# ydchen0806/CLC

Hardware: AMD Instinct MI355X
Metric: images/sec fwd+bwd @256x256 bs8; bpp+PSNR parity vs ref (higher is better)
Workload: dtype f32

## Files before the change

clc_amd/csrc/conv_igemm.hip:

```cpp
#include "common.h"
#ifndef CLC_PF32
#define CLC_PF32 3
#endif

namespace {
#include "conv_common.h"
template <int BM, int BN, int WM, int WN, bool TR>
__global__ __launch_bounds__(64 * WM * WN, (64 * WM * WN) >= 512 ? 4 : ((64 * WM * WN) >= 256 ? 2 : 4))
void conv_igemm_kernel(const ConvParams p) {
  constexpr int NT = 64 * WM * WN;
  constexpr int TM = BM / WM / 32, TN = BN / WN / 32;
  constexpr int A_P = BM * 8 / NT, B_P = BN * 8 / NT;
  static_assert(TM >= 1 && TN >= 1 && A_P * NT == BM * 8 && B_P * NT == BN * 8, "tile");
  extern __shared__ __attribute__((aligned(16))) float smem[];
  float* As = smem;
  float* Bs = smem + 2 * BM * LD;

  const int tid = threadIdx.x, lane = tid & 63, wave = tid >> 6;
  const int wm = wave / WN, wn = wave % WN;
  const int m0 = blockIdx.x * BM, n0 = blockIdx.y * BN;
  const int cls = blockIdx.z, ph = cls >> 1, pw = cls & 1;
  const bool half = p.transposed && p.stride == 2;
  const int DH = half ? p.OH / 2 : p.OH, DW = half ? p.OW / 2 : p.OW;
  const TapGrid tg = make_taps(p, ph, pw);
// ... 431 lines not shown
    dma_a(buf ^ 1); dma_b(buf ^ 1);
    __builtin_amdgcn_s_setprio(0);
    read_frag(buf, 1, af[1], bf[1]);
    mfma_group(af[0], bf[0]);
    read_frag(buf, 2, af[0], bf[0]);
    mfma_group(af[1], bf[1]);
    read_frag(buf, 3, af[1], bf[1]);
    mfma_group(af[0], bf[0]);
    mfma_group(af[1], bf[1]);
    asm volatile("s_waitcnt vmcnt(0)" ::: "memory");
    __syncthreads();
    read_frag(buf ^ 1, 0, af[0], bf[0]);
  }

  if (ksp > 1) {
    float* dst = p.partial + ((size_t)(cls * ksp + sk) * p.M) * p.Cout;
#pragma unroll
    for (int i = 0; i < TM; ++i)
#pragma unroll
      for (int j = 0; j < TN; ++j) {
        const int co = n0 + wn * (BN / WN) + j * 32 + lr;
        const int row0 = m0 + wm * (BM / WM) + i * 32 + 4 * hh;
        if (co >= p.Cout) continue;
#pragma unroll
        for (int r = 0; r < 16; ++r) dst[(size_t)(row0 + (r & 3) + 8 * (r >> 2)) * p.Cout + co] = acc[i][j][r];
      }
    return;
  }
  if (p.reg_epi) {
    const RegEpi re = make_reg_epi(p);
#pragma unroll
    for (int i = 0; i < TM; ++i)
#pragma unroll
      for (int j = 0; j < TN; ++j) {
        const int co = n0 + wn * (BN / WN) + j * 32 + lr;
        epilogue_regs(p, re, acc[i][j], bsel ? bsel[co] : 0.f, (unsigned)(m0 + wm * (BM / WM) + i * 32 + 4 * hh), co);
      }
    return;
  }
  constexpr int LDC = BN + 4;
  float* Cs = smem;
  __syncthreads();
  {
    const int col = lane & 31, rhalf = 4 * (lane >> 5);
#pragma unroll
    for (int i = 0; i < TM; ++i)
#pragma unroll
      for (int j = 0; j < TN; ++j)
#pragma unroll
        for (int r = 0; r < 16; ++r)
          Cs[(wm * (BM / WM) + i * 32 + (r & 3) + 8 * (r >> 2) + rhalf) * LDC + wn * (BN / WN) + j * 32 + col] = acc[i][j][r];
  }
  __syncthreads();
  if (p.vec_epi) {
    for (int e = tid; e < BM * BN / 4; e += NT) {
      const int row = e / (BN / 4), cc = (e - row * (BN / 4)) * 4;
      const int m = m0 + row, co = n0 + cc;
      if (m < p.M && co < p.Cout) epilogue_store4(p, bsel, *reinterpret_cast<const f32x4*>(Cs + row * LDC + cc), m, co, DH, DW, ph, pw);
    }
    return;
  }
  for (int e = tid; e < BM * BN; e += NT) {
    const int row = e / BN, cc = e - row * BN;
    const int m = m0 + row, co = n0 + cc;
    if (m < p.M && co < p.Cout) epilogue_store(p, Cs[row * LDC + cc], bsel ? bsel[co] : 0.f, m, co, DH, DW, ph, pw);
  }
}

template <int KS>
__global__ __launch_bounds__(256, 2)
void conv_igemm_n16_kernel(const ConvParams p) {
  constexpr int BM = 256, NT = 256, A_P = 8;
  extern __shared__ __attribute__((aligned(16))) float smem[];
  float* As = smem;
  float* Bs = smem + 2 * BM * BK;
  const int tid = threadIdx.x, lane = tid & 63, wave = tid >> 6;
  const int m0 = blockIdx.x * BM;
  const int DH = p.OH, DW = p.OW;
  const __amdgpu_buffer_rsrc_t xr = __builtin_amdgcn_make_buffer_rsrc(const_cast<float*>(p.x), 0, p.x_bytes, 0x00020000);
  const __amdgpu_buffer_rsrc_t wr = __builtin_amdgcn_make_buffer_rsrc(const_cast<float*>(p.w), 0, p.w_bytes, 0x00020000);
  unsigned a_base[A_P], a_mask[A_P];
  int a_c4[A_P];
#pragma unroll
  for (int i = 0; i < A_P; ++i) {
    const int r = (tid + i * NT) >> 3;
    const RowState rs = make_row<false>(p, m0 + r, DH, DW, 0, 0);
    a_c4[i] = ((tid & 7) ^ ((r >> 1) & 7)) * 4;
    unsigned mask = 0;
#pragma unroll
    for (int j = 0; j < KS; ++j)
#pragma unroll
      for (int q = 0; q < KS; ++q) {
        const int iy = rs.y0 + j, ix = rs.x0 + q;
        mask |= (rs.ok && (unsigned)iy < (unsigned)p.H && (unsigned)ix < (unsigned)p.W) ? (1u << (j * 3 + q)) : 0u;
      }
    a_mask[i] = mask;
    a_base[i] = ((unsigned)(rs.base + rs.y0 * p.W + rs.x0) * (unsigned)p.ldx + (unsigned)a_c4[i]) * 4u;
  }
  const int b_r = tid >> 3, b_c4 = ((tid & 7) ^ ((b_r >> 1) & 7)) * 4;
  const bool b_ok = tid < 128 && b_r < p.Cout;
  const unsigned b_base = ((unsigned)b_r * (unsigned)p.ldw + (unsigned)b_c4) * 4u;
  const int wave_row = wave * 8;

  f32x4 acc[4];
#pragma unroll
  for (int rb = 0; rb < 4; ++rb) acc[rb] = (f32x4){0.f, 0.f, 0.f, 0.f};
  const int total = KS * KS * p.kc_tiles;
  int tj = 0, ti = 0, kc = 0;
  auto advance = [&]() {
    const int kc1 = kc + 1;
    const bool w1 = kc1 == p.kc_tiles;
    kc = w1 ? 0 : kc1;
    const int ti1 = ti + (w1 ? 1 : 0);
    const bool w2 = ti1 == KS;
    ti = w2 ? 0 : ti1;
    tj += w2 ? 1 : 0;
  };
  unsigned s_bit, s_adelta, s_bdelta; int s_cleft; bool s_en;
  auto set_fetch = [&](bool en) {
    s_en = en;
    s_bit = 1u << (tj * 3 + ti);
    s_cleft = p.Cin - kc * BK;
    s_adelta = (unsigned)((tj * p.W + ti) * p.ldx + kc * BK) * 4u;
    s_bdelta = (unsigned)((tj * KS + ti) * p.Cin + kc * BK) * 4u;
  };
  auto dma_tile = [&](int buf) {
#pragma unroll
    for (int i = 0; i < A_P; ++i) {
      const bool ok = s_en && (a_mask[i] & s_bit) != 0u && a_c4[i] < s_cleft;
      dma16(xr, As + (buf * BM + wave_row + i * (NT / 8)) * BK, ok ? a_base[i] + s_adelta : kOOB);
    }
    if (wave < 2) dma16(wr, Bs + (buf * 16 + wave_row) * BK, (s_en && b_ok && b_c4 < s_cleft) ? b_base + s_bdelta : kOOB);
  };
  set_fetch(true);
  dma_tile(0);
  asm volatile("s_waitcnt vmcnt(0)" ::: "memory");
  __syncthreads();
  const int li = lane & 15, g = lane >> 4, sw = (li >> 1) & 7;
  int fo[2];
#pragma unroll
  for (int t = 0; t < 2; ++t) fo[t] = ((4 * t + g) ^ sw) * 4;
  for (int it = 0; it < total; ++it) {
    const int buf = it & 1;
    advance();
    set_fetch(it + 1 < total);
    dma_tile(buf ^ 1);
    const float* Ab = As + (buf * BM + wave * 64 + li) * BK;
    const float* Bb = Bs + (buf * 16 + li) * BK;
#pragma unroll
    for (int t = 0; t < 2; ++t) {
      f32x4 a[4];
#pragma unroll
      for (int rb = 0; rb < 4; ++rb) a[rb] = *reinterpret_cast<const f32x4*>(Ab + rb * 16 * BK + fo[t]);
      const f32x4 b = *reinterpret_cast<const f32x4*>(Bb + fo[t]);
#pragma unroll
      for (int s = 0; s < 4; ++s)
#pragma unroll
        for (int rb = 0; rb < 4; ++rb) acc[rb] = __builtin_amdgcn_mfma_f32_16x16x4f32(a[rb][s], b[s], acc[rb], 0, 0, 0);
    }
    asm volatile("s_waitcnt vmcnt(0)" ::: "memory");
    __syncthreads();
  }
  const int co = li;
  if (co < p.Cout) {
    const float bv = p.bias ? p.bias[co] : 0.f;
#pragma unroll
    for (int rb = 0; rb < 4; ++rb)
#pragma unroll
      for (int r = 0; r < 4; ++r) {
        const int m = m0 + wave * 64 + rb * 16 + 4 * g + r;
        if (m < p.M) epilogue_store(p, acc[rb][r], bv, m, co, DH, DW, 0, 0);
      }
  }
}

__device__ __forceinline__ void wait_vm(int n) {
  if (n >= 63) asm volatile("s_waitcnt vmcnt(63) lgkmcnt(0)" ::: "memory");
  else if (n == 35) asm volatile("s_waitcnt vmcnt(35) lgkmcnt(0)" ::: "memory");
  else if (n == 19) asm volatile("s_waitcnt vmcnt(19) lgkmcnt(0)" ::: "memory");
  else asm volatile("s_waitcnt vmcnt(3) lgkmcnt(0)" ::: "memory");
}
template <int OP>
__global__ __launch_bounds__(512, 4)
void conv_igemm_p1x1_kernel(const ConvParams p, int tiles_m, int tiles_n) {
  constexpr int BM = 128, BN = 64, NT = 512, NS = 3, SLOT = (BM + BN) * BK;
  constexpr int P = 3;
  extern __shared__ __attribute__((aligned(16))) float smem[];
  const int tid = threadIdx.x, lane = tid & 63, wave = tid >> 6;
  const int wm = wave >> 1, wn = wave & 1;
  const int G = gridDim.x;
  const __amdgpu_buffer_rsrc_t xr = __builtin_amdgcn_make_buffer_rsrc(const_cast<float*>(p.x), 0, p.x_bytes, 0x00020000);
  const __amdgpu_buffer_rsrc_t wr = __builtin_amdgcn_make_buffer_rsrc(const_cast<float*>(p.w), 0, p.w_bytes, 0x00020000);

  unsigned a_lane[2], b_lane;
  int a_c4[2], b_c4;
#pragma unroll
  for (int i = 0; i < 2; ++i) {
    const int r = (tid + i * NT) >> 3;
    a_c4[i] = ((tid & 7) ^ ((r >> 1) & 7)) * 4;
    a_lane[i] = ((unsigned)r * (unsigned)p.ldx + (unsigned)a_c4[i]) * 4u;
  }
  {
    const int r = tid >> 3;
    b_c4 = ((tid & 7) ^ ((r >> 1) & 7)) * 4;
    b_lane = ((unsigned)r * (unsigned)p.ldw + (unsigned)b_c4) * 4u;
  }
  const int wave_row = wave * 8;
  float* bias_s = smem + NS * SLOT;
  for (int i = tid; i < p.Cout; i += NT) bias_s[i] = p.bias ? p.bias[i] : 0.f;
  const int my_mt = (tiles_m - (int)blockIdx.x + G - 1) / G;
  const int total = my_mt * tiles_n * p.kc_tiles;

  struct Cur { int mt, nt, kt, n; };
  auto step = [&](Cur& c) {
    const int kt1 = c.kt + 1;
    const bool w1 = kt1 == p.kc_tiles;
    c.kt = w1 ? 0 : kt1;
    const int nt1 = c.nt + (w1 ? 1 : 0);
    const bool w2 = nt1 == tiles_n;
    c.nt = w2 ? 0 : nt1;
    c.mt += w2 ? G : 0;
    ++c.n;
  };
  auto dma = [&](int slot, const Cur& c) {
    const bool en = c.n < total;
    const int cleft = p.Cin - c.kt * BK;
    const unsigned ao = ((unsigned)(c.mt * BM) * (unsigned)p.ldx + (unsigned)(c.kt * BK)) * 4u;
    const unsigned bo = ((unsigned)(c.nt * BN) * (unsigned)p.ldw + (unsigned)(c.kt * BK)) * 4u;
    float* base = smem + slot * SLOT;
#pragma unroll
    for (int i = 0; i < 2; ++i) dma16(xr, base + (wave_row + i * 64) * BK, (en && a_c4[i] < cleft) ? a_lane[i] + ao : kOOB);
    dma16(wr, base + (BM + wave_row) * BK, (en && b_c4 < cleft) ? b_lane + bo : kOOB);
  };

  const int lr = lane & 31, hh = lane >> 5, sw = (lr >> 1) & 7;
  int fo[4];
#pragma unroll
  for (int t8 = 0; t8 < 4; ++t8) fo[t8] = ((2 * t8 + hh) ^ sw) * 4;
  f32x4 af[2], bf[2];
  auto read_frag = [&](int slot, int t8, f32x4& a, f32x4& b) {
    const float* base = smem + slot * SLOT;
    a = *reinterpret_cast<const f32x4*>(base + (wm * 32 + lr) * BK + fo[t8]);
    if (OP == 1) a = a * a;
    b = *reinterpret_cast<const f32x4*>(base + (BM + wn * 32 + lr) * BK + fo[t8]);
  };
  f32x16 acc;
#pragma unroll
  for (int r = 0; r < 16; ++r) acc[r] = 0.f;
  auto mfma4 = [&](const f32x4& a, const f32x4& b) {
#pragma unroll
    for (int ss = 0; ss < 4; ++ss) acc = __builtin_amdgcn_mfma_f32_32x32x2f32(a[ss], b[ss], acc, 0, 0, 0);
  };

  const RegEpi re = make_reg_epi(p);
  const int S = p.y_pre ? 32 : 16;
  auto epilogue = [&](int mt, int nt) {
    const int co = nt * BN + wn * 32 + lr;
    epilogue_regs(p, re, acc, bias_s[co], (unsigned)(mt * BM + wm * 32 + 4 * hh), co);
  };


  Cur cf{(int)blockIdx.x, 0, 0, 0}, cc = cf;
  dma(0, cf); step(cf);
  dma(1, cf); step(cf);
  asm volatile("s_waitcnt vmcnt(3) lgkmcnt(0)" ::: "memory");
  __builtin_amdgcn_s_barrier();
  int slot = 0, slot2 = 2, e_prev = 0;
  for (int s = 0; s < total; ++s) {
    dma(slot2, cf); step(cf);
    read_frag(slot, 0, af[0], bf[0]);
    read_frag(slot, 1, af[1], bf[1]);
    mfma4(af[0], bf[0]);
    read_frag(slot, 2, af[0], bf[0]);
    mfma4(af[1], bf[1]);
    read_frag(slot, 3, af[1], bf[1]);
    mfma4(af[0], bf[0]);
    mfma4(af[1], bf[1]);
    const bool last = cc.kt == p.kc_tiles - 1;
    if (last) {
      epilogue(cc.mt, cc.nt);
#pragma unroll
      for (int r = 0; r < 16; ++r) acc[r] = 0.f;
    }
    const int e_cur = last ? 1 : 0;
    wait_vm(P + S * (e_prev + e_cur));
    __builtin_amdgcn_s_barrier();
    e_prev = e_cur;
    step(cc);
    slot = slot == 2 ? 0 : slot + 1;
    slot2 = slot2 == 2 ? 0 : slot2 + 1;
  }
  asm volatile("s_waitcnt vmcnt(0)" ::: "memory");
}

template <int BN, bool TR, int KW, int PF, bool OPS>
__global__ __launch_bounds__(64 * KW, KW == 8 ? (PF >= 2 ? 1 : 4) : 4)
void conv_igemm_splitk_kernel(const ConvParams p) {
  constexpr int BM = 32, TN = BN / 32;
  extern __shared__ __attribute__((aligned(16))) float smem[];
  const int tid = threadIdx.x, lane = tid & 63, wave = tid >> 6;
  const int li = lane & 31, h = lane >> 5;

  const int m0 = blockIdx.x * BM, n0 = blockIdx.y * BN;
  const int cls = blockIdx.z, ph = cls >> 1, pw = cls & 1;
  const bool half = p.transposed && p.stride == 2;
  const int DH = half ? p.OH / 2 : p.OH, DW = half ? p.OW / 2 : p.OW;
  const TapGrid tg = make_taps(p, ph, pw);

  const int fset = p.group_rows ? min(m0 / p.group_rows, 3) : 0;
  const float* wsel = fset == 0 ? p.w : (fset == 1 ? p.w2 : (fset == 2 ? p.w3 : p.w4));
  const float* bsel = fset == 0 ? p.bias : (fset == 1 ? p.bias2 : (fset == 2 ? p.bias3 : p.bias4));
  const __amdgpu_buffer_rsrc_t xr = __builtin_amdgcn_make_buffer_rsrc(const_cast<float*>(p.x), 0, p.x_bytes, 0x00020000);
  const __amdgpu_buffer_rsrc_t wr = __builtin_amdgcn_make_buffer_rsrc(const_cast<float*>(wsel), 0, p.w_bytes, 0x00020000);

  const RowState row = make_row<TR>(p, m0 + li, DH, DW, ph, pw);
  unsigned b_row_off[TN];
  bool b_ok[TN];
#pragma unroll
  for (int j = 0; j < TN; ++j) {
    const int co = n0 + j * 32 + li;
    b_ok[j] = co < p.Cout;
    b_row_off[j] = (unsigned)co * (unsigned)p.ldw;
  }
  const bool sq = OPS && p.in_op == CLC_IN_SQUARE;
  const int total = tg.nkh * tg.nkw * p.kc_tiles;

  const bool fuse_act = OPS && p.xs != nullptr;
  const __amdgpu_buffer_rsrc_t sr = __builtin_amdgcn_make_buffer_rsrc(const_cast<float*>(fuse_act ? p.xs : p.x), 0, fuse_act ? p.xs_bytes : p.x_bytes, 0x00020000);
  f32x4 af[PF][4], sf[PF][4], bf[PF][TN][4];
  auto load_tile = [&](int slot, int it) {
    const int t = it / p.kc_tiles, kc = it - t * p.kc_tiles;
    const int tj = t / tg.nkw, ti = t - tj * tg.nkw;
    const int kh = tg.kh0 + tg.step * tj, kw = tg.kw0 + tg.step * ti;
    const unsigned tap_off = (unsigned)((kh * p.ks + kw) * p.Cin);
    const unsigned pix = a_pixel<TR>(p, row, kh, kw);
#pragma unroll
    for (int t8 = 0; t8 < 4; ++t8) {
      const int c = kc * BK + t8 * 8 + 4 * h;
      const bool c_ok = c < p.Cin;
      af[slot][t8] = buf_load4(xr, pix_off(pix, p.ldx, c, c_ok));
      if (OPS && fuse_act) sf[slot][t8] = buf_load4(sr, pix_off(pix, p.ldxs, c, c_ok));
#pragma unroll
      for (int j = 0; j < TN; ++j) bf[slot][j][t8] = buf_load4(wr, (b_ok[j] && c_ok) ? (b_row_off[j] + tap_off + (unsigned)c) * 4u : kOOB);
    }
  };

  f32x16 acc[TN];
#pragma unroll
  for (int j = 0; j < TN; ++j)
#pragma unroll
    for (int r = 0; r < 16; ++r) acc[j][r] = 0.f;

#pragma unroll
  for (int s = 0; s < PF; ++s)
    if (wave + s * KW < total) load_tile(s, wave + s * KW);
  int it = wave;
  for (int base = 0; it < total; base += PF) {
#pragma unroll
    for (int s = 0; s < PF; ++s) {
      if (it < total) {
#pragma unroll
        for (int t8 = 0; t8 < 4; ++t8) {
          f32x4 a = af[s][t8];
          if constexpr (OPS) {
            if (sq) a = a * a;
            if (fuse_act) a = a * act_deriv4(sf[s][t8], p.xs_act, p.xs_pre);
          }
#pragma unroll
          for (int ss = 0; ss < 4; ++ss)
#pragma unroll
            for (int j = 0; j < TN; ++j) acc[j] = __builtin_amdgcn_mfma_f32_32x32x2f32(a[ss], bf[s][j][t8][ss], acc[j], 0, 0, 0);
        }
        if (it + PF * KW < total) load_tile(s, it + PF * KW);
      }
      it += KW;
    }
  }

  float* red = smem;
#pragma unroll
  for (int j = 0; j < TN; ++j)
#pragma unroll
    for (int r = 0; r < 16; ++r) red[((wave * TN + j) * 16 + r) * 64 + lane] = acc[j][r];
  __syncthreads();
  if (p.vec_epi) {
    for (int e = tid; e < BM * BN / 4; e += 64 * KW) {
      const int rowi = e / (BN / 4), cc = (e - rowi * (BN / 4)) * 4;
      const int j = cc >> 5, r = (rowi & 3) + 4 * (rowi >> 3), ln = (cc & 31) + 32 * ((rowi >> 2) & 1);
      f32x4 q[KW];
#pragma unroll
      for (int w = 0; w < KW; ++w) q[w] = *reinterpret_cast<const f32x4*>(red + ((w * TN + j) * 16 + r) * 64 + ln);
      f32x4 v = (q[0] + q[1]) + (q[2] + q[3]);
      if constexpr (KW == 8) v = v + ((q[4] + q[5]) + (q[6] + q[7]));
      const int m = m0 + rowi, co = n0 + cc;
      if (m < p.M && co < p.Cout) epilogue_store4(p, bsel, v, m, co, DH, DW, ph, pw);
    }
    return;
  }
  for (int e = tid; e < BM * BN; e += 64 * KW) {
    const int rowi = e / BN, cc = e - rowi * BN;
    const int j = cc >> 5, r = (rowi & 3) + 4 * (rowi >> 3), ln = (cc & 31) + 32 * ((rowi >> 2) & 1);
    float q[KW];
#pragma unroll
    for (int w = 0; w < KW; ++w) q[w] = red[((w * TN + j) * 16 + r) * 64 + ln];
    float v = (q[0] + q[1]) + (q[2] + q[3]);
    if constexpr (KW == 8) v = v + ((q[4] + q[5]) + (q[6] + q[7]));
    const int m = m0 + rowi, co = n0 + cc;
    if (m < p.M && co < p.Cout) epilogue_store(p, v, bsel ? bsel[co] : 0.f, m, co, DH, DW, ph, pw);
  }
}

__global__ __launch_bounds__(256) void conv_splitk_finish_kernel(const ConvParams p, int classes) {
  const int c4n = p.Cout >> 2;
  const long per_class = (long)p.M * c4n, total = per_class * classes;
  const bool half = p.transposed && p.stride == 2;
  const int DH = half ? p.OH / 2 : p.OH, DW = half ? p.OW / 2 : p.OW;
  for (long i = (long)blockIdx.x * blockDim.x + threadIdx.x; i < total; i += (long)gridDim.x * blockDim.x) {
    const int cls = (int)(i / per_class);
    const long r = i - (long)cls * per_class;
    const int m = (int)(r / c4n), co = (int)(r - (long)m * c4n) * 4;
    const float* src = p.partial + ((size_t)(cls * p.ksplit) * p.M + m) * p.Cout + co;
    f32x4 acc = *reinterpret_cast<const f32x4*>(src);
    for (int s2 = 1; s2 < p.ksplit; ++s2) acc = acc + *reinterpret_cast<const f32x4*>(src + (size_t)s2 * p.M * p.Cout);
    const int fset = p.group_rows ? min(m / p.group_rows, 3) : 0;
    const float* bsel = fset == 0 ? p.bias : (fset == 1 ? p.bias2 : (fset == 2 ? p.bias3 : p.bias4));
    epilogue_store4(p, bsel, acc, m, co, DH, DW, cls >> 1, cls & 1);
  }
}
static int heavy128_split(const ConvParams& p, int classes) {
  if (!clc_tuning[CLC_TUNE_HEAVY128] || !p.batch_variant_ok || p.transposed || !p.vec_epi || p.in_op != CLC_IN_NONE || p.xs || p.shuffle || classes != 1) return 1;
  if (p.ks != 3 || p.stride != 1 || p.OH * p.OW > 256 || p.Cout < 128 || p.Cout % 32 || p.M % 128 || p.M < 2048) return 1;
  const int ksteps = 9 * p.kc_tiles;
  if (ksteps < 108) return 1;
  const long wgs = (long)(p.M / 128) * ((p.Cout + 127) / 128);
  int k = (int)((256 + wgs - 1) / wgs);
  if (k > 8) k = 8;
  while (k > 1 && ksteps / k < 16) --k;
  return k;
}
static int conv_ksplit(const ConvParams& p, int classes) {
  { const int k128 = heavy128_split(p, classes); if (k128 > 1) return k128; }
  if (!clc_tuning[CLC_TUNE_DGRAD_SPLITK] || !p.transposed || !p.vec_epi || p.in_op != CLC_IN_NONE || p.xs || p.shuffle) return 1;
  if (p.M % 64 || p.Cout % 64) return 1;
  const long wgs = (long)(p.M / 64) * (p.Cout / 64) * classes;
  const int ksteps = (p.transposed && p.stride == 2 ? ((p.ks + 1) / 2) * ((p.ks + 1) / 2) : p.ks * p.ks) * p.kc_tiles;
  const int min_steps = clc_tuning[CLC_TUNE_DGRAD_SPLITK] > 1 ? clc_tuning[CLC_TUNE_DGRAD_SPLITK] : 56;
  if (wgs >= 384 || ksteps < min_steps) return 1;
  int k = (int)((640 + wgs - 1) / wgs);
  if (k > 4) k = 4;
  while (k > 1 && ksteps / k < 24) --k;
  return k;
}

template <int BM, int BN, int WM, int WN, bool TR>
int launch_t(const ConvParams& p, int classes, hipStream_t st) {
  dim3 grid((p.M + BM - 1) / BM, (p.Cout + BN - 1) / BN, classes);
  const size_t lds = (size_t)2 * (BM + BN) * LD * sizeof(float);
  static_assert(BM * (BN + 4) <= 2 * (BM + BN) * LD, "C tile must fit in the operand tiles' LDS");
  static PerDeviceOnce attr_once;
  if (attr_once.first()) {
    (void)hipFuncSetAttribute(reinterpret_cast<const void*>(&conv_igemm_kernel<BM, BN, WM, WN, TR>), hipFuncAttributeMaxDynamicSharedMemorySize, (int)lds);
  }
  hipLaunchKernelGGL((conv_igemm_kernel<BM, BN, WM, WN, TR>), grid, dim3(64 * WM * WN), lds, st, p);
  CLC_LAUNCH_CHECK();
  return (1 << 20) | (WM << 16) | (WN << 12) | (BM << 3) | (BN >> 5);
}
template <int BM, int BN, int WM, int WN, bool TR>
int launch_dma_t(const ConvParams& p, int classes, hipStream_t st) {
  dim3 grid((p.M + BM - 1) / BM, (p.Cout + BN - 1) / BN, classes);
  constexpr size_t lds_ab = (size_t)2 * (BM + BN) * BK * sizeof(float), lds_c = (size_t)BM * (BN + 4) * sizeof(float);
  constexpr size_t lds = lds_ab > lds_c ? lds_ab : lds_c;
  static PerDeviceOnce attr_once;
  if (attr_once.first()) {
    (void)hipFuncSetAttribute(reinterpret_cast<const void*>(&conv_igemm_dma_kernel<BM, BN, WM, WN, TR>), hipFuncAttributeMaxDynamicSharedMemorySize, (int)lds);
  }
  hipLaunchKernelGGL((conv_igemm_dma_kernel<BM, BN, WM, WN, TR>), grid, dim3(64 * WM * WN), lds, st, p);
  CLC_LAUNCH_CHECK();
  return (2 << 20) | (WM << 16) | (WN << 12) | (BM << 3) | (BN >> 5);
}
template <int BM, int BN, int WM, int WN, bool TR, int KS, int OP = 0, bool BF = false>
int launch_dma2_t(const ConvParams& p, int classes, hipStream_t st) {
  dim3 grid((p.M + BM - 1) / BM, (p.Cout + BN - 1) / BN, classes);
  constexpr size_t lds_ab = (size_t)2 * (BM + BN) * BK * sizeof(float), lds_c = (size_t)BM * (BN + 4) * sizeof(float);
  constexpr size_t lds = lds_ab > lds_c ? lds_ab : lds_c;
  static PerDeviceOnce attr_once;
  if (attr_once.first()) {
    (void)hipFuncSetAttribute(reinterpret_cast<const void*>(&conv_igemm_dma2_kernel<BM, BN, WM, WN, TR, KS, OP, BF>), hipFuncAttributeMaxDynamicSharedMemorySize, (int)lds);
  }
  ConvParams q = p;
  const int xm = clc_tuning[CLC_TUNE_XCD_MAP];
  q.xcd_map = grid.y > 1 && grid.x % 8 == 0 && (xm == 2 || (xm == 1 && KS == 1));
  q.reg_epi = clc_tuning[CLC_TUNE_REG_EPI] && reg_epi_ok(p, BM, BN);
  if (p.ksplit > 1) {
    grid.z = classes * p.ksplit;
    q.xcd_map = 0;
  }
  hipLaunchKernelGGL((conv_igemm_dma2_kernel<BM, BN, WM, WN, TR, KS, OP, BF>), grid, dim3(64 * WM * WN), lds, st, q);
  CLC_LAUNCH_CHECK();
  if (p.ksplit > 1) {
    const long total = (long)p.M * (p.Cout / 4) * classes;
    long nb = (total + 255) / 256;
    if (nb > 4096) nb = 4096;
    hipLaunchKernelGGL(conv_splitk_finish_kernel, dim3((unsigned)nb), dim3(256), 0, st, q, classes);
    CLC_LAUNCH_CHECK();
  }
  return ((KS == 1 ? 5 : 4) << 20) | (OP << 24) | ((BF ? 1 : 0) << 26) | (WM << 16) | (WN << 12) | (BM << 3) | (BN >> 5);
}
int launch_n16(const ConvParams& p, int classes, hipStream_t st) {
  if (!clc_tuning[CLC_TUNE_N16] || classes != 1 || p.transposed || p.stride != 1 || p.Cout > 16 || p.group_rows || p.xs || p.in_op != CLC_IN_NONE || p.ksplit > 1) return 0;
  if (p.ks != 3) return 0;
  dim3 grid((p.M + 255) / 256);
  const size_t lds = (size_t)2 * (256 + 16) * BK * sizeof(float);
  static PerDeviceOnce attr_once;
  if (attr_once.first()) (void)hipFuncSetAttribute(reinterpret_cast<const void*>(&conv_igemm_n16_kernel<3>), hipFuncAttributeMaxDynamicSharedMemorySize, (int)lds);
  hipLaunchKernelGGL((conv_igemm_n16_kernel<3>), grid, dim3(256), lds, st, p);
  CLC_LAUNCH_CHECK();
  return (10 << 20) | (4 << 16) | (256 << 3);
}
int launch_p1x1(const ConvParams& p, int classes, hipStream_t st) {
  if (!clc_tuning[CLC_TUNE_P1X1] || classes != 1 || p.ks != 1 || p.stride != 1 || p.shuffle || p.group_rows || p.xs) return 0;
  if (p.M % 128 || p.Cout % 64 || p.kc_tiles < 2 || !(p.in_op == CLC_IN_NONE || p.in_op == CLC_IN_SQUARE)) return 0;
  const int tiles_m = p.M / 128, tiles_n = p.Cout / 64;
  if (!reg_epi_ok(p, 128, 64)) return 0;
  if (tiles_m < (clc_tuning[CLC_TUNE_P1X1] >= 2 ? 256 : 512)) return 0;
  const size_t lds = (size_t)3 * (128 + 64) * BK * sizeof(float) + (size_t)p.Cout * sizeof(float);
  if (lds > 80 * 1024) return 0;
  const int grid = tiles_m < 512 ? tiles_m : 512;
  static PerDeviceOnce attr_once;
  if (attr_once.first()) {
    (void)hipFuncSetAttribute(reinterpret_cast<const void*>(&conv_igemm_p1x1_kernel<0>), hipFuncAttributeMaxDynamicSharedMemorySize, 80 * 1024);
    (void)hipFuncSetAttribute(reinterpret_cast<const void*>(&conv_igemm_p1x1_kernel<1>), hipFuncAttributeMaxDynamicSharedMemorySize, 80 * 1024);
  }
  if (p.in_op == CLC_IN_SQUARE) hipLaunchKernelGGL((conv_igemm_p1x1_kernel<1>), dim3(grid), dim3(512), lds, st, p, tiles_m, tiles_n);
  else hipLaunchKernelGGL((conv_igemm_p1x1_kernel<0>), dim3(grid), dim3(512), lds, st, p, tiles_m, tiles_n);
  CLC_LAUNCH_CHECK();
  return (8 << 20) | ((p.in_op == CLC_IN_SQUARE ? 1 : 0) << 24) | (4 << 16) | (2 << 12) | (128 << 3) | (64 >> 5);
}
template <int BM, int BN, int WM, int WN>
int launch(const ConvParams& p, int classes, hipStream_t st) {
  static const int use_dma = getenv("CLC_DMA") ? atoi(getenv("CLC_DMA")) : 1;
  static const int dma_small = getenv("CLC_DMA_SMALL") ? atoi(getenv("CLC_DMA_SMALL")) : 1;
  if (use_dma && p.in_op == CLC_IN_SQUARE && p.xs == nullptr && p.ks == 1 && p.stride == 1 && (BM >= 128 || dma_small) && clc_tuning[CLC_TUNE_DMA_LOOP] == 2)
    return p.transposed ? launch_dma2_t<BM, BN, WM, WN, true, 1, 1>(p, classes, st) : launch_dma2_t<BM, BN, WM, WN, false, 1, 1>(p, classes, st);
  if (use_dma && p.in_op == CLC_IN_NONE && p.xs == nullptr && (BM >= 128 || dma_small) && clc_tuning[CLC_TUNE_DMA_LOOP] == 2)
    return p.ks == 1 && p.stride == 1
               ? (p.transposed ? launch_dma2_t<BM, BN, WM, WN, true, 1>(p, classes, st) : launch_dma2_t<BM, BN, WM, WN, false, 1>(p, classes, st))
               : (p.bf16
                      ? (p.transposed ? launch_dma2_t<BM, BN, WM, WN, true, 3, 0, true>(p, classes, st) : launch_dma2_t<BM, BN, WM, WN, false, 3, 0, true>(p, classes, st))
                      : (p.transposed ? launch_dma2_t<BM, BN, WM, WN, true, 3>(p, classes, st) : launch_dma2_t<BM, BN, WM, WN, false, 3>(p, classes, st)));
  if (use_dma && p.in_op == CLC_IN_NONE && p.xs == nullptr && (BM >= 128 || dma_small))
    return p.transposed ? launch_dma_t<BM, BN, WM, WN, true>(p, classes, st) : launch_dma_t<BM, BN, WM, WN, false>(p, classes, st);
  return p.transposed ? launch_t<BM, BN, WM, WN, true>(p, classes, st) : launch_t<BM, BN, WM, WN, false>(p, classes, st);
}

template <int BN, bool TR, int KW, int PF, bool OPS>
int launch_splitk_t(const ConvParams& p, int classes, hipStream_t st) {
  dim3 grid((p.M + 31) / 32, (p.Cout + BN - 1) / BN, classes);
  const size_t lds = (size_t)KW * (BN / 32) * 16 * 64 * sizeof(float);
  static PerDeviceOnce attr_once;
  if (attr_once.first()) {
    (void)hipFuncSetAttribute(reinterpret_cast<const void*>(&conv_igemm_splitk_kernel<BN, TR, KW, PF, OPS>), hipFuncAttributeMaxDynamicSharedMemorySize, (int)lds);
  }
  hipLaunchKernelGGL((conv_igemm_splitk_kernel<BN, TR, KW, PF, OPS>), grid, dim3(64 * KW), lds, st, p);
  CLC_LAUNCH_CHECK();
  return (3 << 20) | (KW << 16) | (32 << 3) | (BN >> 5);
}
template <int BN, bool TR, int KW, int PF>
int launch_splitk_o(const ConvParams& p, int classes, hipStream_t st) {
  return (p.xs != nullptr || p.in_op == CLC_IN_SQUARE) ? launch_splitk_t<BN, TR, KW, PF, true>(p, classes, st) : launch_splitk_t<BN, TR, KW, PF, false>(p, classes, st);
}
template <int BN>
int launch_splitk(const ConvParams& p, int classes, hipStream_t st) {
  static const int kw4 = getenv("CLC_SPLITK_KW4") ? atoi(getenv("CLC_SPLITK_KW4")) : 1;
  if (kw4 && p.ks * p.ks * p.kc_tiles <= 4)
    return p.transposed ? launch_splitk_o<BN, true, 4, 1>(p, classes, st) : launch_splitk_o<BN, false, 4, 1>(p, classes, st);
  if (clc_tuning[CLC_TUNE_SPLITK_PF] == 1)
    return p.transposed ? launch_splitk_o<BN, true, 8, 1>(p, classes, st) : launch_splitk_o<BN, false, 8, 1>(p, classes, st);
  return p.transposed ? launch_splitk_o<BN, true, 8, 3>(p, classes, st) : launch_splitk_o<BN, false, 8, 3>(p, classes, st);
}

__global__ void conv_direct_small_kernel(const ConvParams p) {
  const long idx = (long)blockIdx.x * blockDim.x + threadIdx.x;
  const int cgroups = (p.Cout + 3) / 4;
  const long total = (long)p.M * cgroups;
  if (idx >= total) return;
  const int cg = (int)(idx % cgroups);
  const int m = (int)(idx / cgroups);
  const int n = m / (p.OH * p.OW), rr = m - n * (p.OH * p.OW);
  const int oy = rr / p.OW, ox = rr - oy * p.OW;
  float acc[4] = {0.f, 0.f, 0.f, 0.f};
  for (int kh = 0; kh < p.ks; ++kh) {
    const int iy = oy * p.stride - p.pad + kh;
    if (iy < 0 || iy >= p.H) continue;
    for (int kw = 0; kw < p.ks; ++kw) {
      const int ix = ox * p.stride - p.pad + kw;
      if (ix < 0 || ix >= p.W) continue;
      const float* xp = p.x + (size_t)((n * p.H + iy) * p.W + ix) * p.ldx;
      for (int ci = 0; ci < p.Cin; ++ci) {
        float xv = xp[ci];
        if (p.in_op == CLC_IN_SQUARE) xv *= xv;
#pragma unroll
        for (int q = 0; q < 4; ++q) {
          const int co = cg * 4 + q;
          if (co < p.Cout) acc[q] = fmaf(xv, p.w[(size_t)co * p.ldw + (kh * p.ks + kw) * p.Cin + ci], acc[q]);
        }
      }
    }
  }
#pragma unroll
  for (int q = 0; q < 4; ++q) {
    const int co = cg * 4 + q;
    if (co < p.Cout) epilogue_store(p, acc[q], p.bias ? p.bias[co] : 0.f, m, co, p.OH, p.OW, 0, 0);
  }
}

__global__ void filter_transpose_kernel(const float* __restrict__ w, float* __restrict__ wt, int Cout, int T, int Cin) {
  __shared__ float tile[32][33];
  const int t = blockIdx.z;
  const int co0 = blockIdx.y * 32, ci0 = blockIdx.x * 32;
  const int tx = threadIdx.x & 31, ty = threadIdx.x >> 5;
  for (int r = ty; r < 32; r += 8) {
    const int co = co0 + r, ci = ci0 + tx;
    tile[r][tx] = (co < Cout && ci < Cin) ? w[((size_t)co * T + t) * Cin + ci] : 0.f;
  }
  __syncthreads();
  for (int r = ty; r < 32; r += 8) {
    const int ci = ci0 + r, co = co0 + tx;
    if (ci < Cin && co < Cout) wt[((size_t)ci * T + t) * Cout + co] = tile[tx][r];
  }
}

__global__ void filter_transpose_batched_kernel(const clc_transpose_entry* __restrict__ table, int n_entries) {
  __shared__ float tile[32][33];
  int lo = 0, hi = n_entries - 1;
  const int b = blockIdx.x;
  while (lo < hi) {
    const int mid = (lo + hi + 1) >> 1;
    if (table[mid].tile_begin <= b) lo = mid; else hi = mid - 1;
  }
  const clc_transpose_entry e = table[lo];
  const int nci = (e.Cin + 31) / 32, nco = (e.Cout + 31) / 32;
  int local = b - e.tile_begin;
  const int t = local / (nci * nco); local -= t * nci * nco;
  const int co0 = (local / nci) * 32, ci0 = (local % nci) * 32;
  const int tx = threadIdx.x & 31, ty = threadIdx.x >> 5;
  for (int r = ty; r < 32; r += 8) {
    const int co = co0 + r, ci = ci0 + tx;
    tile[r][tx] = (co < e.Cout && ci < e.Cin) ? e.w[((size_t)co * e.T + t) * e.Cin + ci] : 0.f;
  }
  __syncthreads();
  for (int r = ty; r < 32; r += 8) {
    const int ci = ci0 + r, co = co0 + tx;
    if (ci < e.Cin && co < e.Cout) e.wt[((size_t)ci * e.T + t) * e.Cout + co] = tile[tx][r];
  }
}

}

extern "C" int clc_filter_transpose_batched(const clc_transpose_entry* table_dev, int n_entries, int total_tiles, clc_stream_t stream) {
  CLC_CHECK(table_dev && n_entries > 0 && total_tiles > 0, "clc_filter_transpose_batched: bad args");
  hipLaunchKernelGGL(filter_transpose_batched_kernel, dim3(total_tiles), dim3(256), 0, (hipStream_t)stream, table_dev, n_entries);
  CLC_LAUNCH_CHECK();
  return 0;
}

static void use_split(ConvParams& p, const clc_conv_desc* d, int classes) {
  const int k = conv_ksplit(p, classes);
  if (k > 1 && d->workspace && d->workspace_bytes >= (size_t)k * classes * p.M * p.Cout * sizeof(float) && aligned16(d->workspace) &&
      clc_tuning[CLC_TUNE_DMA_LOOP] == 2) {
    p.ksplit = k;
    p.partial = (float*)d->workspace;
  }
}

static int fill_params(const clc_conv_desc* d, ConvParams& p, int& classes) {
  CLC_CHECK(d && d->x && d->w && d->y, "clc_conv2d: null pointer");
  CLC_CHECK(d->ks == 1 || d->ks == 3, "clc_conv2d: ks must be 1 or 3 (got %d)", d->ks);
  CLC_CHECK(d->stride == 1 || d->stride == 2, "clc_conv2d: stride must be 1 or 2 (got %d)", d->stride);
  CLC_CHECK(d->N > 0 && d->H > 0 && d->W > 0 && d->Cin > 0 && d->Cout > 0 && d->OH > 0 && d->OW > 0, "clc_conv2d: bad dims");
  CLC_CHECK(d->ldx >= d->Cin, "clc_conv2d: ldx < Cin");
  if (!d->transposed) {
    CLC_CHECK(d->OH == (d->H + 2 * d->pad - d->ks) / d->stride + 1 && d->OW == (d->W + 2 * d->pad - d->ks) / d->stride + 1,
              "clc_conv2d: output dims %dx%d inconsistent with input %dx%d ks=%d s=%d pad=%d", d->OH, d->OW, d->H, d->W, d->ks, d->stride, d->pad);
  } else {
    CLC_CHECK(d->H == (d->OH + 2 * d->pad - d->ks) / d->stride + 1 && d->W == (d->OW + 2 * d->pad - d->ks) / d->stride + 1,
              "clc_conv2d(transposed): dY dims %dx%d inconsistent with dX %dx%d", d->H, d->W, d->OH, d->OW);
    CLC_CHECK(d->stride == 1 || (d->OH % 2 == 0 && d->OW % 2 == 0), "clc_conv2d(transposed,s2): odd dX dims");
    CLC_CHECK(!d->shuffle, "clc_conv2d: shuffle with transposed");
  }
  CLC_CHECK(!d->shuffle || d->Cout % 4 == 0, "clc_conv2d: shuffle needs Cout %% 4 == 0");
  CLC_CHECK(d->norm == CLC_NORM_NONE || d->mul, "clc_conv2d: norm without mul");
  const int och = d->shuffle ? d->Cout / 4 : d->Cout;
  CLC_CHECK(d->ldy >= och, "clc_conv2d: ldy < channels");
  const size_t x_bytes = ((size_t)d->N * d->H * d->W - 1) * d->ldx * 4 + (size_t)d->Cin * 4;
  const size_t w_bytes = (size_t)d->Cout * d->ks * d->ks * d->Cin * 4;
  CLC_CHECK(x_bytes < (1ull << 31) && w_bytes < (1ull << 31), "clc_conv2d: tensor larger than 2 GiB");
  CLC_CHECK((size_t)d->N * d->OH * d->OW * (d->shuffle ? 4 : 1) < (1ull << 31), "clc_conv2d: too many pixels");

  p.x = d->x; p.w = d->w; p.bias = d->bias; p.y = d->y; p.mul = d->mul; p.res = d->res; p.y_pre = d->y_pre;
  p.N = d->N; p.H = d->H; p.W = d->W; p.Cin = d->Cin; p.ldx = d->ldx;
  p.OH = d->OH; p.OW = d->OW; p.Cout = d->Cout; p.ldy = d->ldy;
  p.ks = d->ks; p.stride = d->stride; p.pad = d->pad; p.transposed = d->transposed; p.in_op = d->in_op;
  p.act = d->act; p.norm = d->norm; p.shuffle = d->shuffle; p.res_first = d->res_first;
  p.ldm = d->ldm; p.ldr = d->ldr; p.ldp = d->ldp; p.ldw = d->ks * d->ks * d->Cin; p.res_scale = d->res_scale;
  p.kc_tiles = (d->Cin + BK - 1) / BK;
  p.x_bytes = (unsigned)x_bytes; p.w_bytes = (unsigned)w_bytes;
  p.xs = d->xs; p.ldxs = d->ldxs; p.xs_act = d->xs_act; p.xs_pre = d->xs_pre; p.xs_bytes = 0;
  if (d->xs) {
    CLC_CHECK(d->ldxs >= d->Cin && d->ldxs % 4 == 0 && aligned16(d->xs), "clc_conv2d: bad xs (fused activation backward operand)");
    const size_t sb = ((size_t)d->N * d->H * d->W - 1) * d->ldxs * 4 + (size_t)d->Cin * 4;
    CLC_CHECK(sb < (1ull << 31), "clc_conv2d: xs larger than 2 GiB");
    p.xs_bytes = (unsigned)sb;
  }
  {
    auto ok4 = [](const void* ptr, int ld) { return ptr == nullptr || (aligned16(ptr) && ld % 4 == 0); };
    p.vec_epi = !d->shuffle && d->Cout % 4 == 0 && ok4(d->y, d->ldy) && ok4(d->res, d->ldr) && ok4(d->mul, d->ldm) && ok4(d->y_pre, d->ldp) && ok4(d->res_gate, d->ldg) && ok4(d->out_gate, d->ldog);
  }
  classes = 1;
  p.M = d->N * d->OH * d->OW;
  if (d->transposed && d->stride == 2) { classes = 4; p.M = d->N * (d->OH / 2) * (d->OW / 2); }
  p.w2 = d->w2; p.bias2 = d->bias2; p.group_rows = 0; p.pre_deriv = d->pre_deriv;
  p.dma_place = clc_tuning[CLC_TUNE_DMA_PLACE]; p.xcd_map = 0; p.ablate = clc_tuning[CLC_TUNE_ABLATE]; p.reg_epi = 0; p.ksplit = 1; p.partial = nullptr; p.batch_variant_ok = d->batch_variant_ok; p.bf16 = 0;
  p.res_gate = d->res ? d->res_gate : nullptr; p.ldg = d->ldg; p.rg_act = d->res_gate_act; p.rg_pre = d->res_gate_pre;
  p.out_gate = d->out_gate; p.ldog = d->ldog; p.og_act = d->out_gate_act; p.og_pre = d->out_gate_pre;
  CLC_CHECK(!d->out_gate || !d->shuffle, "clc_conv2d: out_gate with shuffle");
  p.w3 = d->w3; p.bias3 = d->bias3; p.w4 = d->w4; p.bias4 = d->bias4;
  if (d->w2) {
    const int sets = d->w3 ? 4 : 2;
    CLC_CHECK((d->w3 != nullptr) == (d->w4 != nullptr), "clc_conv2d: w3 and w4 must be given together");
    CLC_CHECK(d->N % sets == 0, "clc_conv2d: %d filter sets need a batch that is a multiple of %d (got N=%d)", sets, sets, d->N);
    CLC_CHECK((d->bias == nullptr) == (d->bias2 == nullptr) && (!d->w3 || ((d->bias == nullptr) == (d->bias3 == nullptr) && (d->bias == nullptr) == (d->bias4 == nullptr))),
              "clc_conv2d: the bias must be given for every filter set or for none");
    CLC_CHECK(aligned16(d->w2) && (!d->w3 || (aligned16(d->w3) && aligned16(d->w4))) && (d->Cin % 4 == 0) && (d->ldx % 4 == 0),
              "clc_conv2d: filter sets need the aligned (Cin %% 4 == 0) path");
    p.group_rows = p.M / sets;
    CLC_CHECK(p.group_rows % 128 == 0, "clc_conv2d: filter sets need (N/sets)*rows-per-image to be a multiple of the largest tile (128), got %d", p.group_rows);
  } else {
    CLC_CHECK(!d->w3 && !d->w4, "clc_conv2d: w3 / w4 without w2");
  }

  return 0;
}

extern "C" size_t clc_conv2d_workspace_bytes(const clc_conv_desc* d) {
  if (!d) return 0;
  ConvParams p;
  int classes = 1;
  if (fill_params(d, p, classes) < 0) return 0;
  const bool vec_ok = (d->Cin % 4 == 0) && (d->ldx % 4 == 0) && aligned16(d->x) && aligned16(d->w);
  if (!vec_ok || d->Cout < 64) return 0;
  const int img_pix = (d->transposed && d->stride == 2) ? (d->OH / 2) * (d->OW / 2) : d->OH * d->OW;
  if (img_pix > 1024) return 0;
  const int k = conv_ksplit(p, classes);
  return k > 1 ? (size_t)k * classes * p.M * p.Cout * sizeof(float) : 0;
}

extern "C" int clc_conv2d(const clc_conv_desc* d, clc_stream_t stream) {
  hipStream_t st = (hipStream_t)stream;
  ConvParams p;
  int classes = 1;
  if (fill_params(d, p, classes) < 0) return -1;
  const bool vec_ok = (d->Cin % 4 == 0) && (d->ldx % 4 == 0) && aligned16(d->x) && aligned16(d->w);
  if (!vec_ok) {
    CLC_CHECK(!d->transposed && !d->xs, "clc_conv2d: unaligned/small-Cin path has no transposed / fused-activation mode (Cin=%d ldx=%d)", d->Cin, d->ldx);
    const int cgroups = (d->Cout + 3) / 4;
    const long total = (long)p.M * cgroups;
    hipLaunchKernelGGL(conv_direct_small_kernel, dim3((unsigned)((total + 255) / 256)), dim3(256), 0, st, p);
    CLC_LAUNCH_CHECK();
    return 1;
  }
  const int img_pix = (d->transposed && d->stride == 2) ? (d->OH / 2) * (d->OW / 2) : d->OH * d->OW;
  const int C = d->Cout;
  const int splitk_pix = clc_tuning[CLC_TUNE_SPLITK_PIX] > 0 ? clc_tuning[CLC_TUNE_SPLITK_PIX] : 256;
  const bool small_map = img_pix <= 256 || (img_pix <= splitk_pix && C <= clc_tuning[CLC_TUNE_SPLITK_MAXC]);
  if (small_map) {
    if (heavy128_split(p, classes) > 1) {
      use_split(p, d, classes);
      if (p.ksplit > 1) return launch<128, 128, 4, 2>(p, classes, st);
    }
    static const int heavy_dgrad = getenv("CLC_HEAVY_DGRAD") ? atoi(getenv("CLC_HEAVY_DGRAD")) : 1;
    static const int heavy_min = getenv("CLC_HEAVY_MIN") ? atoi(getenv("CLC_HEAVY_MIN")) : 60;
    if (heavy_dgrad && img_pix <= 256 && d->transposed && d->ks * d->ks * p.kc_tiles >= heavy_min && C >= 128 &&
        (long)((p.M + 63) / 64) * ((C + 63) / 64) * classes >= 128) {
      use_split(p, d, classes);
      return launch<64, 64, 2, 2>(p, classes, st);
    }
    static const int sk_rule = getenv("CLC_SPLITK_RULE") ? atoi(getenv("CLC_SPLITK_RULE")) : 1;
    if (sk_rule == 0) {
      if ((long)d->Cout * d->ks * d->ks * d->Cin > 200000 && C > 32) return launch_splitk<64>(p, classes, st);
      return launch_splitk<32>(p, classes, st);
    }
    const long wg32 = (long)((p.M + 31) / 32) * ((C + 31) / 32) * classes;
    if (C > 32 && wg32 > 256) return launch_splitk<64>(p, classes, st);
    return launch_splitk<32>(p, classes, st);
  }
  p.bf16 = clc_tuning[CLC_TUNE_BF16] != 0 && img_pix > 256;
  if ((clc_tuning[CLC_TUNE_WINO] & (d->transposed ? 2 : 1)) && d->w_wino && d->ks == 3 && d->stride == 1 && classes == 1) {
    const int v = clc_conv_wino_launch(&p, d->w_wino, st);
    if (v) return v;
  }
  if (clc_tuning[CLC_TUNE_HALO] && d->w_packed && d->ks == 3 && d->stride == 1 && classes == 1) {
    const int v = clc_conv_halo_launch(&p, d->w_packed, st);
    if (v) return v;
  }
  if (img_pix <= 1024) {
    if (C >= 64) {
      use_split(p, d, classes);
      return launch<64, 64, 2, 2>(p, classes, st);
    }
    return launch<64, 32, 2, 1>(p, classes, st);
  }
  if (clc_tuning[CLC_TUNE_LIN] && d->ks == 1 && d->stride == 1 && classes == 1 && vec_ok && !p.shuffle && !p.group_rows && !p.xs && p.in_op == CLC_IN_NONE &&
      p.act == CLC_ACT_NONE && p.norm == CLC_NORM_NONE && !p.y_pre && !p.res_gate && !p.out_gate && p.ldw == p.Cin && p.vec_epi && !p.bf16) {
    const int v = clc_lin_launch(p.x, p.ldx, p.w, p.bias, p.res, p.ldr, p.res_scale, p.y, p.ldy, p.M, p.Cin, p.Cout, st);
    if (v) { CLC_LAUNCH_CHECK(); return v; }
  }
  if (d->ks == 1 && C > 32 && vec_ok) {
    const int v = launch_p1x1(p, classes, st);
    if (v) return v;
  }
  if (clc_tuning[CLC_TUNE_1X1_TILE] && d->ks == 1 && p.kc_tiles <= clc_tuning[CLC_TUNE_1X1_TILE] && C > 32) return launch<128, 64, 4, 2>(p, classes, st);
  if (C % 128 == 0 || C >= 384) return launch<128, 128, 4, 2>(p, classes, st);
  if (clc_tuning[CLC_TUNE_TILE256] && d->ks == 3 && C > 32 && C <= 64 && p.M >= 256 * 512 && (!p.group_rows || p.group_rows % 256 == 0))
    return launch<256, 64, 4, 2>(p, classes, st);
  if (C > 32) return launch<128, 64, 4, 2>(p, classes, st);
  if (C <= 16 && vec_ok) {
    const int v = launch_n16(p, classes, st);
    if (v) return v;
  }
  if (clc_tuning[CLC_TUNE_TILE256] && d->ks == 3 && p.M % 128 == 0 && p.M >= 128 * 512) return launch<128, 32, 2, 1>(p, classes, st);
  return launch<64, 32, 2, 1>(p, classes, st);
}

extern "C" int clc_filter_transpose(const float* w, float* wt, int Cout, int T, int Cin, clc_stream_t stream) {
  CLC_CHECK(w && wt && Cout > 0 && T > 0 && Cin > 0, "clc_filter_transpose: bad args");
  dim3 grid((Cin + 31) / 32, (Cout + 31) / 32, T);
  hipLaunchKernelGGL(filter_transpose_kernel, grid, dim3(256), 0, (hipStream_t)stream, w, wt, Cout, T, Cin);
  CLC_LAUNCH_CHECK();
  return 0;
}
```

Baseline: 341.3.

## Split 8-wave split-K conv kernel into two 4-wave workgroups with partial reduction

For small-image convolutions with many K tiles and few output tiles, the 8-wave split-K kernel is relaunched as two 4-wave workgroups per tile. Each workgroup handles half of the interleaved K chains and writes its partial sum to a workspace, and a separate finish kernel adds the two partials and applies the epilogue. The aim is more workgroups in flight to fill CUs on low-parallelism layers. The cost is extra global traffic for the partials, a second kernel launch, and a larger workspace requirement.

```diff
diff --git a/clc_amd/csrc/conv_igemm.hip b/clc_amd/csrc/conv_igemm.hip
--- a/clc_amd/csrc/conv_igemm.hip
+++ b/clc_amd/csrc/conv_igemm.hip
@@ -757,7 +757,10 @@
   const int li = lane & 31, h = lane >> 5;
 
   const int m0 = blockIdx.x * BM, n0 = blockIdx.y * BN;
-  const int cls = blockIdx.z, ph = cls >> 1, pw = cls & 1;
+  const bool split = KW == 8 && p.ksplit > 1;
+  const int part = split ? (int)blockIdx.z & 1 : 0;
+  const int cls = split ? (int)blockIdx.z >> 1 : (int)blockIdx.z, ph = cls >> 1, pw = cls & 1;
+  const int chain = wave + part * 4;
   const bool half = p.transposed && p.stride == 2;
   const int DH = half ? p.OH / 2 : p.OH, DW = half ? p.OW / 2 : p.OW;
   const TapGrid tg = make_taps(p, ph, pw);
@@ -808,8 +811,8 @@
 
 #pragma unroll
   for (int s = 0; s < PF; ++s)
-    if (wave + s * KW < total) load_tile(s, wave + s * KW);
-  int it = wave;
+    if (chain + s * KW < total) load_tile(s, chain + s * KW);
+  int it = chain;
   for (int base = 0; it < total; base += PF) {
 #pragma unroll
     for (int s = 0; s < PF; ++s) {
@@ -838,6 +841,20 @@
 #pragma unroll
     for (int r = 0; r < 16; ++r) red[((wave * TN + j) * 16 + r) * 64 + lane] = acc[j][r];
   __syncthreads();
+  if (split) {
+    float* dst = p.partial + (size_t)(cls * 2 + part) * p.M * p.Cout;
+    for (int e = tid; e < BM * BN / 4; e += 64 * 4) {
+      const int rowi = e / (BN / 4), cc = (e - rowi * (BN / 4)) * 4;
+      const int j = cc >> 5, r = (rowi & 3) + 4 * (rowi >> 3), ln = (cc & 31) + 32 * ((rowi >> 2) & 1);
+      f32x4 q[4];
+#pragma unroll
+      for (int w = 0; w < 4; ++w) q[w] = *reinterpret_cast<const f32x4*>(red + ((w * TN + j) * 16 + r) * 64 + ln);
+      const f32x4 v = (q[0] + q[1]) + (q[2] + q[3]);
+      const int m = m0 + rowi, co = n0 + cc;
+      if (m < p.M && co < p.Cout) *reinterpret_cast<f32x4*>(dst + (size_t)m * p.Cout + co) = v;
+    }
+    return;
+  }
   if (p.vec_epi) {
     for (int e = tid; e < BM * BN / 4; e += 64 * KW) {
       const int rowi = e / (BN / 4), cc = (e - rowi * (BN / 4)) * 4;
@@ -1016,8 +1033,17 @@
   if (attr_once.first()) {
     (void)hipFuncSetAttribute(reinterpret_cast<const void*>(&conv_igemm_splitk_kernel<BN, TR, KW, PF, OPS>), hipFuncAttributeMaxDynamicSharedMemorySize, (int)lds);
   }
-  hipLaunchKernelGGL((conv_igemm_splitk_kernel<BN, TR, KW, PF, OPS>), grid, dim3(64 * KW), lds, st, p);
+  const bool split = KW == 8 && p.ksplit > 1;
+  if (split) grid.z = classes * 2;
+  hipLaunchKernelGGL((conv_igemm_splitk_kernel<BN, TR, KW, PF, OPS>), grid, dim3(split ? 64 * 4 : 64 * KW), lds, st, p);
   CLC_LAUNCH_CHECK();
+  if (split) {
+    const long total = (long)p.M * (p.Cout / 4) * classes;
+    long nb = (total + 255) / 256;
+    if (nb > 4096) nb = 4096;
+    hipLaunchKernelGGL(conv_splitk_finish_kernel, dim3((unsigned)nb), dim3(256), 0, st, p, classes);
+    CLC_LAUNCH_CHECK();
+  }
   return (3 << 20) | (KW << 16) | (32 << 3) | (BN >> 5);
 }
 template <int BN, bool TR, int KW, int PF>
@@ -1126,6 +1152,14 @@
     p.ksplit = k;
     p.partial = (float*)d->workspace;
   }
+}
+
+static int splitk_chain_split(const ConvParams& p, int classes) {
+  static const int v2 = getenv("CLC_SPLITK_V2") ? atoi(getenv("CLC_SPLITK_V2")) : 1;
+  if (!v2 || !p.vec_epi || p.shuffle) return 1;
+  const int ktiles = (p.transposed && p.stride == 2 ? ((p.ks + 1) / 2) * ((p.ks + 1) / 2) : p.ks * p.ks) * p.kc_tiles;
+  const long tiles = (long)((p.M + 31) / 32) * ((p.Cout + 31) / 32) * classes;
+  return ktiles >= 48 && tiles < 256 ? 2 : 1;
 }
 
 static int fill_params(const clc_conv_desc* d, ConvParams& p, int& classes) {
@@ -1207,7 +1241,10 @@
   const int img_pix = (d->transposed && d->stride == 2) ? (d->OH / 2) * (d->OW / 2) : d->OH * d->OW;
   if (img_pix > 1024) return 0;
   const int k = conv_ksplit(p, classes);
-  return k > 1 ? (size_t)k * classes * p.M * p.Cout * sizeof(float) : 0;
+  const size_t s64 = k > 1 ? (size_t)k * classes * p.M * p.Cout * sizeof(float) : 0;
+  const int c = img_pix <= 256 ? splitk_chain_split(p, classes) : 1;
+  const size_t s32 = c > 1 ? (size_t)c * classes * p.M * p.Cout * sizeof(float) : 0;
+  return s64 > s32 ? s64 : s32;
 }
 
 extern "C" int clc_conv2d(const clc_conv_desc* d, clc_stream_t stream) {
@@ -1247,6 +1284,11 @@
     }
     const long wg32 = (long)((p.M + 31) / 32) * ((C + 31) / 32) * classes;
     if (C > 32 && wg32 > 256) return launch_splitk<64>(p, classes, st);
+    if (img_pix <= 256 && splitk_chain_split(p, classes) == 2 && d->workspace && aligned16(d->workspace) &&
+        d->workspace_bytes >= (size_t)2 * classes * p.M * p.Cout * sizeof(float)) {
+      p.ksplit = 2;
+      p.partial = (float*)d->workspace;
+    }
     return launch_splitk<32>(p, classes, st);
   }
   p.bf16 = clc_tuning[CLC_TUNE_BF16] != 0 && img_pix > 256;
```

Result: no change. 343.0, median of 6 (+0.5%).
